# foolwood/SiamMask

Hardware: NVIDIA H100
Metric: search-region frames/sec (127/255 SiamMask-sharp) (higher is better)
Workload: dtype f16x3 (hi+lo split fp16 operands on wgmma, f32 accumulate; f32 CUDA-core xcorr/refine)

## Files before the change

siammask_b200/build.py:

```python
from __future__ import annotations

import os
import shutil
import subprocess
import sys

HERE = os.path.dirname(os.path.abspath(__file__))
CSRC = os.path.join(HERE, "csrc")
LIB = os.path.join(HERE, "libsiammask_b200.so")
SOURCES = ["conv_gemm_sm90.cu", "conv3x3_patch_sm90.cu", "stem_sm90.cu", "simt_kernels.cu", "xcorr_bulk.cu", "engine.cu"]
HEADERS = ["common.cuh", "ptx.cuh", os.path.join("..", "..", "include", "siammask_b200.h")]
NVCC_FLAGS = ["-gencode", "arch=compute_90a,code=sm_90a", "-lineinfo", "-O3", "-std=c++17",
              "-Xcompiler", "-fPIC", "-shared"]


def _nvcc() -> str:
    for cand in (os.environ.get("NVCC"), shutil.which("nvcc"), "/usr/local/cuda/bin/nvcc"):
        if cand and os.path.exists(cand):
            return cand
    raise RuntimeError("nvcc not found; cannot build libsiammask_b200.so")


HASH = LIB + ".srchash"


def source_hash() -> str:
    import hashlib
    h = hashlib.sha256(" ".join(NVCC_FLAGS).encode())
    for d in SOURCES + HEADERS:
        path = os.path.join(CSRC, d)
        h.update(d.encode())
        if os.path.exists(path):
            with open(path, "rb") as f:
                h.update(f.read())
    return h.hexdigest()


def is_stale() -> bool:
    if not os.path.exists(LIB):
        return True
    try:
        with open(HASH) as f:
            return f.read().strip() != source_hash()
    except OSError:
        return True


def build(force: bool = False, verbose: bool = False) -> str:
    if not force and not is_stale():
        return LIB
    tmp = f"{LIB}.tmp{os.getpid()}"
    cmd = [_nvcc(), *NVCC_FLAGS, "-o", tmp, *[os.path.join(CSRC, s) for s in SOURCES]]
    if verbose:
        print(" ".join(cmd), file=sys.stderr)
    digest = source_hash()
    res = subprocess.run(cmd, capture_output=True, text=True)
    if res.returncode != 0:
        if os.path.exists(tmp):
            os.remove(tmp)
        raise RuntimeError("nvcc failed:\n" + res.stdout + res.stderr)
    os.replace(tmp, LIB)
    with open(f"{HASH}.tmp{os.getpid()}", "w") as f:
        f.write(digest + "\n")
    os.replace(f"{HASH}.tmp{os.getpid()}", HASH)
    return LIB


if __name__ == "__main__":
    print(build(force="--force" in sys.argv, verbose=True))
```

siammask_b200/csrc/common.cuh:

```cuda
#pragma once
#include <cuda.h>
#include <cuda_fp16.h>
#include <cuda_runtime.h>
#include <cstdint>
#include <cstdio>
#include <stdexcept>
#include <string>
#include <vector>

struct sm_image_desc;

namespace smk {

struct Act {
  __half* hi = nullptr;
  __half* lo = nullptr;
  int B = 0, H = 0, W = 0, C = 0;
  int sexp = 0;
  __host__ __device__ size_t numel() const { return (size_t)B * H * W * C; }
  __host__ __device__ int M() const { return B * H * W; }
};

struct ConvGeom {
  int Cin, Cout, KH, KW, stride, pad, dil;
  __host__ __device__ int out_size(int in) const { return (in + 2 * pad - dil * (KH - 1) - 1) / stride + 1; }
};

enum OutMode : int { OUT_NHWC_SPLIT = 0, OUT_NHWC_F32 = 1, OUT_NCHW_F32 = 2 };

struct Epilogue {
  const float* alpha = nullptr;
  const float* beta = nullptr;
  const __half* res_hi = nullptr;
  const __half* res_lo = nullptr;
  float res_scale = 1.f;
  __half* out_hi = nullptr;
  __half* out_lo = nullptr;
  float* out_f32 = nullptr;
  int out_mode = OUT_NHWC_SPLIT;
  int relu = 0;
  int* ovf = nullptr;
};

__device__ __forceinline__ void flag_if_out_of_range(float absmax, int* ovf) {
  if (ovf != nullptr && !(absmax <= 65504.f)) atomicOr(ovf, 1);
}
constexpr int kStatusBadSlot = 2;

struct GemmSegment {
  CUtensorMap tmA[2];
  int mode;
  int num_kb, cblks, KW;
  int stride, pad, dil;
  int b_col0;
};

struct GemmParams {
  GemmSegment seg[2];
  int nseg;
  CUtensorMap tmB[2];
  CUtensorMap tmO[2];
  CUtensorMap tmR[2];
  int has_res;
  int M, Cout, Ho, Wo;
  int n_tiles, m_tiles;
  int reverse_m;
  Epilogue ep;
};

struct GemmInput {
  Act in;
  ConvGeom g;
  int w_col0;
};

struct TrackerHp {
  double context_amount, penalty_k, window_influence, lr;
  int32_t exemplar_size, instance_size, total_stride, base_size, out_size, reserved;
};

struct CudaError : std::runtime_error {
  using std::runtime_error::runtime_error;
};

#define SMK_CUDA(expr)                                                                              \
  do {                                                                                              \
    cudaError_t _e = (expr);                                                                        \
    if (_e != cudaSuccess)                                                                          \
      throw smk::CudaError(std::string(#expr) + " failed: " + cudaGetErrorString(_e) + " at " +    \
                           __FILE__ + ":" + std::to_string(__LINE__));                              \
  } while (0)

#define SMK_CHECK(cond, msg)                                                                        \
  do {                                                                                              \
    if (!(cond)) throw std::runtime_error(std::string("check failed: ") + #cond + " — " + (msg));   \
  } while (0)

template <typename K>
inline void ensure_dynamic_smem(K kernel, int bytes, unsigned long long& done_mask) {
  int dev = 0;
  SMK_CUDA(cudaGetDevice(&dev));
  const unsigned long long bit = 1ull << (dev & 63);
  if (done_mask & bit) return;
  SMK_CUDA(cudaFuncSetAttribute(kernel, cudaFuncAttributeMaxDynamicSharedMemorySize, bytes));
  done_mask |= bit;
}


bool gemm_conv_supported(const ConvGeom& g);
void launch_gemm_conv(const Act& in, const ConvGeom& g, const __half* w_hi, const __half* w_lo, int cout_pad,
                      const Epilogue& ep, int nsplit, int num_sms, cudaStream_t st);
void launch_gemm_multi(const GemmInput* convs, int nconv, const Act* residual, const __half* w_hi,
                       const __half* w_lo, int cout_pad, int w_ld, const Epilogue& ep, int nsplit, int num_sms,
                       cudaStream_t st, bool reverse_m = false);

CUtensorMap make_map_tiled_nd(const __half* base, int rank, const uint64_t* dims, const uint64_t* strides_bytes,
                              const uint32_t* box, int swizzle_bytes);

bool patch_conv_supported(const Act& in, const ConvGeom& g);
void launch_conv3x3_patch(const Act& in, const ConvGeom& g, const __half* w_hi, const __half* w_lo, int w_ld,
                          const Epilogue& ep, int nsplit, int num_sms, cudaStream_t st);

void launch_stem_tc(const float* x_nchw, int B, int S, const __half* w_hi, const __half* w_lo, const float* alpha,
                    const float* beta, Act out, int num_sms, cudaStream_t st, int* ovf = nullptr);

void launch_ref_conv(const Act& in, const ConvGeom& g, const float* w_krsc_cout, const Epilogue& ep,
                     cudaStream_t st);
void launch_stem(const float* x_nchw, int B, int S, const float* w, const float* alpha, const float* beta, Act out,
                 cudaStream_t st);
void launch_maxpool3s2(const Act& in, Act out, cudaStream_t st);
void launch_xcorr_nhwc(const Act& x, int c_off, const __half* k_hi, const __half* k_lo, int kh, int kw, Act out,
                       float mul, int* ovf, cudaStream_t st, const int32_t* slots = nullptr, int num_slots = 0);
void launch_scatter_slots(const __half* src_hi, const __half* src_lo, __half* dst_hi, __half* dst_lo,
                          const int32_t* slots, int B, int num_slots, int n, int* status, cudaStream_t st);
void launch_paste_labels(const float* masks, int side, const double* maps, const uint8_t* anno, const int32_t* obj_off,
                         const int32_t* objects, int G, int H, int W, double seg_thr, uint8_t* labels, cudaStream_t st,
                         const sm_image_desc* desc = nullptr);
void launch_paste_labels_iou(const float* masks, int side, const double* maps, const uint8_t* anno,
                             const int32_t* obj_off, const int32_t* objects, const int32_t* target_ids, int G, int H,
                             int W, double seg_thr, uint8_t* labels, const double* thrs, int T, int32_t* counts,
                             cudaStream_t st, const sm_image_desc* desc = nullptr);
void launch_label_boxes(const uint8_t* anno, int G, int H, int W, const int32_t* queries, int Q, int32_t* boxes,
                        cudaStream_t st, const sm_image_desc* desc = nullptr);
void launch_vot_overlap(const float* poly_a, const float* poly_b, int B, int W, int H, float* overlap, cudaStream_t st,
                        const int32_t* wh = nullptr);
void launch_vot_trajectory_overlap(const double* rec, int T, int S, const float* gt, int gt_frames, const int32_t* seq,
                                   const int32_t* wh, const int32_t* lengths, float* acc, float* eao, cudaStream_t st);
size_t vot_eao_workspace_size(int T, int S);
void launch_vot_eao_accumulate(const float* eao, const float* acc, const double* rec, int T, int S,
                               const int32_t* lengths, const int32_t* combo, int R, int cap, int tail_from,
                               const double* tail_in, double* tail_out, double* num, double* den, double* stats,
                               void* workspace, cudaStream_t st);
void launch_absmax(const Act& a, float* slot, cudaStream_t st);
void launch_xcorr_nchw_f32(const float* x, const float* k, float* out, int planes, int H, int W, int kh, int kw,
                           cudaStream_t st);
int launch_xcorr_bulk_f32(const float* x, const float* k, float* out, int planes, int H, int W, int kh, int kw,
                          cudaStream_t st);
void launch_crop_center(const Act& in, int crop, Act out, cudaStream_t st);
void launch_refine_crop(const Act& in, const int32_t* pos, int pos_max, int scale, int padv, int size, Act out,
                        cudaStream_t st);
void launch_gather_corr(const Act& corr, const int32_t* pos, float* out, float mul, cudaStream_t st);
void launch_gather_mask_col(const float* mask, const int32_t* pos, int B, int C, int R, float* out, cudaStream_t st);
void launch_deconv(const float* p3, const float* w, const float* bias, float* out, int B, int Cin, int N,
                   int cout, cudaStream_t st);
void launch_split_to_f32(const Act& in, float* out, cudaStream_t st, float mul = 1.f);
void launch_import_nchw(const float* x_nchw, Act out, cudaStream_t st);
void launch_warp_affine(const float* src, int sh, int sw, const double* maps, float* dst, int dh, int dw, float border,
                        int B, cudaStream_t st, const sm_image_desc* dst_desc = nullptr);
void launch_tracker_prepare(int B, const double* state, const int32_t* avg, const TrackerHp& hp, int32_t* boxes,
                            double* tsz, double* aux, cudaStream_t st);
void launch_tracker_update(int B, double* state, const float* rec, const double* aux, const int32_t* imsize,
                           const TrackerHp& hp, int A, int R, double* maps, double* out, cudaStream_t st,
                           const double* hp_table = nullptr);
void launch_crop_resize(const uint8_t* frames, size_t frame_stride, int H, int W, const int32_t* box, int B, int model,
                        float* out, cudaStream_t st, const int32_t* frame_idx = nullptr,
                        const sm_image_desc* desc = nullptr);
void launch_select(const float* cls, const float* loc, const float* anchors, const float* window, const double* tsz,
                   int B, int A, int R, double penalty_k, double window_influence, int32_t* best_idx, int32_t* pos,
                   float* rec, cudaStream_t st, const double* hp = nullptr);
void launch_mask_iou(const float* masks, int side, const double* maps, const uint8_t* anno, const int32_t* video, int B,
                     int H, int W, const double* thrs, int T, int32_t* counts, cudaStream_t st,
                     const sm_image_desc* desc = nullptr);
void launch_small_conv3x3_maps(const float* a, const float* b, int B, int Hi, int Wi, int Ho, int Wo, int Cin, int Cout,
                               const int* ymap, const int* xmap, const float* w, const float* bias, int relu,
                               float* out, cudaStream_t st);
std::vector<int> nearest_index_table(int out_size, int in_size);
int gemm_cout_pad(int cout);

}
```

siammask_b200/csrc/conv_gemm_sm90.cu:

```cuda
#include "common.cuh"
#include "ptx.cuh"

#include <cstdlib>
#include <cstring>
#include <mutex>
#include <unordered_map>

namespace smk {

namespace {

constexpr int BLOCK_M = 128;
constexpr int WG_ROWS = 64;
constexpr int CIN_GRAIN = 64;
constexpr int MMA_K = 16;
constexpr int SMEM_LIMIT = 227 * 1024;
constexpr int NUM_CONSUMER_WARPS = 8;
constexpr int NUM_THREADS = 128 + 32 * NUM_CONSUMER_WARPS;
constexpr int PRODUCER_REGS = 40;
constexpr int CONSUMER_REGS = 232;

template <int BLOCK_N, int NSPLIT>
struct Cfg {
  static constexpr int STAGING_BYTES = WG_ROWS * BLOCK_N * 4;
  static constexpr int RING_BYTES = SMEM_LIMIT - 2048 - 2 * STAGING_BYTES;
  static constexpr int stage_bytes(int bk) { return NSPLIT * (BLOCK_M + BLOCK_N) * bk * 2; }
  static constexpr int BLOCK_K = RING_BYTES / stage_bytes(64) >= 3 ? 64 : 32;
  static constexpr int SW = BLOCK_K * 2;
  static constexpr int A_TILE_BYTES = BLOCK_M * BLOCK_K * 2;
  static constexpr int B_TILE_BYTES = BLOCK_N * BLOCK_K * 2;
  static constexpr int STAGE_BYTES = NSPLIT * (A_TILE_BYTES + B_TILE_BYTES);
  static constexpr int RAW_STAGES = RING_BYTES / STAGE_BYTES;
  static constexpr int STAGES = RAW_STAGES > 6 ? 6 : RAW_STAGES;
  static constexpr int SMEM_BYTES = STAGES * STAGE_BYTES + 2 * STAGING_BYTES + 1024  + 256 ;
  static constexpr int ACC = BLOCK_N / 2;
  static constexpr int H_BOX = BLOCK_N < 64 ? BLOCK_N : 64;
  static constexpr int F_BOX = BLOCK_N < 32 ? BLOCK_N : 32;
  static constexpr int H_PLANE = WG_ROWS * BLOCK_N * 2;
  static_assert(STAGES >= 3, "pipeline needs at least three stages");
  static_assert(BLOCK_N % 16 == 0 && BLOCK_N >= 16 && BLOCK_N <= 128, "N tile (register accumulators)");
  static_assert(STAGE_BYTES % 1024 == 0 && B_TILE_BYTES % 1024 == 0, "stage parts stay 1024-aligned (swizzle atoms)");
  static_assert(SMEM_BYTES <= SMEM_LIMIT, "shared memory budget");
};

__device__ __forceinline__ int m_block(const GemmParams& p, int tile) {
  const int mb = tile / p.n_tiles;
  return p.reverse_m ? p.m_tiles - 1 - mb : mb;
}

template <int SPAN>
__device__ __forceinline__ uint32_t swizzle(uint32_t o) {
  return o ^ (((o >> 7) & (SPAN / 16 - 1)) << 4);
}

__device__ __forceinline__ void named_barrier_sync(int id, int threads) {
  asm volatile("bar.sync %0, %1;" ::"r"(id), "r"(threads) : "memory");
}

template <int BLOCK_N, int NSPLIT>
__global__ void __launch_bounds__(NUM_THREADS, 1) conv_gemm_kernel(const __grid_constant__ GemmParams p) {
  using C = Cfg<BLOCK_N, NSPLIT>;
  constexpr int STAGES = C::STAGES;
  constexpr int BLOCK_K = C::BLOCK_K;
  constexpr int A_TILE_BYTES = C::A_TILE_BYTES;

  extern __shared__ uint8_t smem_raw[];
  uint8_t* smem = smem_raw + ((1024u - (smem_u32(smem_raw) & 1023u)) & 1023u);
  uint8_t* staging = smem + STAGES * C::STAGE_BYTES;
  uint64_t* full_bar = reinterpret_cast<uint64_t*>(staging + 2 * C::STAGING_BYTES);
  uint64_t* empty_bar = full_bar + STAGES;
  uint64_t* free_bar = empty_bar + STAGES;
  uint64_t* res_bar = free_bar + 2;

  const int warp = __shfl_sync(0xffffffffu, (int)(threadIdx.x >> 5), 0);
  const int lane = threadIdx.x & 31;
  const int num_tiles = p.m_tiles * p.n_tiles;

  if (threadIdx.x == 0) {
    for (int i = 0; i < NSPLIT; ++i) {
      for (int sgi = 0; sgi < p.nseg; ++sgi) tma_prefetch_desc(&p.seg[sgi].tmA[i]);
      tma_prefetch_desc(&p.tmB[i]);
    }
    for (int s = 0; s < STAGES; ++s) {
      mbar_init(&full_bar[s], 1);
      mbar_init(&empty_bar[s], NUM_CONSUMER_WARPS);
    }
    for (int w = 0; w < 2; ++w) {
      mbar_init(&free_bar[w], 1);
      mbar_init(&res_bar[w], 1);
    }
    fence_barrier_init();
  }
  __syncthreads();

  if (warp < 4) {
    setmaxnreg_dec<PRODUCER_REGS>();
    if (warp != 0) return;
    const bool leader = elect_one();
    int stage = 0;
    uint32_t phase = 0;
    uint32_t iter = 0;
    for (int tile = blockIdx.x; tile < num_tiles; tile += gridDim.x, ++iter) {
      const int m0 = m_block(p, tile) * BLOCK_M;
      const int n0 = (tile % p.n_tiles) * BLOCK_N;
      const int q = m0 % p.Wo;
      const int t = m0 / p.Wo;
      const int pq = t % p.Ho;
      const int nb = t / p.Ho;
      for (int sgi = 0; sgi < p.nseg; ++sgi) {
        const GemmSegment& sg = p.seg[sgi];
        const int wb = q * sg.stride - sg.pad;
        const int hb = pq * sg.stride - sg.pad;
#pragma unroll 1
        for (int kb = 0; kb < sg.num_kb; ++kb) {
          mbar_wait(&empty_bar[stage], phase ^ 1);
          if (leader) mbar_arrive_expect_tx(&full_bar[stage], C::STAGE_BYTES);
          uint8_t* st = smem + stage * C::STAGE_BYTES;
          const int tap = kb / sg.cblks;
          const int c0 = (kb - tap * sg.cblks) * BLOCK_K;
#pragma unroll
          for (int s = 0; s < NSPLIT; ++s) {
            uint8_t* a_dst = st + s * A_TILE_BYTES;
            if (leader) {
              if (sg.mode == 0) {
                tma_load_2d(a_dst, &sg.tmA[s], &full_bar[stage], c0, m0);
              } else {
                const int r = tap / sg.KW;
                const int sx = tap - r * sg.KW;
                tma_load_im2col_4d(a_dst, &sg.tmA[s], &full_bar[stage], c0, wb, hb, nb,
                                   static_cast<uint16_t>(sx * sg.dil), static_cast<uint16_t>(r * sg.dil));
              }
              tma_load_2d(st + NSPLIT * A_TILE_BYTES + s * C::B_TILE_BYTES, &p.tmB[s], &full_bar[stage],
                          sg.b_col0 + kb * BLOCK_K, n0);
            }
          }
          __syncwarp();
          if (++stage == STAGES) { stage = 0; phase ^= 1; }
        }
      }
      if (p.has_res) {
#pragma unroll 1
        for (int w = 0; w < 2; ++w) {
          mbar_wait(&free_bar[w], iter & 1);
          const int r0 = m0 + w * WG_ROWS;
          if (leader) {
            mbar_arrive_expect_tx(&res_bar[w], r0 < p.M ? NSPLIT * C::H_PLANE : 0);
            if (r0 < p.M) {
              uint8_t* dst = staging + w * C::STAGING_BYTES;
#pragma unroll
              for (int s = 0; s < NSPLIT; ++s)
#pragma unroll
                for (int b = 0; b < BLOCK_N / C::H_BOX; ++b)
                  tma_load_2d(dst + s * C::H_PLANE + b * (WG_ROWS * C::H_BOX * 2), &p.tmR[s], &res_bar[w],
                              n0 + b * C::H_BOX, r0);
            }
          }
          __syncwarp();
        }
      }
    }
    return;
  }

  setmaxnreg_inc<CONSUMER_REGS>();
  const int wg = (warp >> 2) - 1;
  const int wl = warp & 3;
  const bool store_thread = wl == 0 && lane == 0;
  const Epilogue& ep = p.ep;
  const int HoWo = p.Ho * p.Wo;
  uint8_t* my_staging = staging + wg * C::STAGING_BYTES;
  float acc[C::ACC];
  float acc2[C::ACC];
  int stage = 0;
  uint32_t phase = 0;
  uint32_t iter = 0;
  for (int tile = blockIdx.x; tile < num_tiles; tile += gridDim.x, ++iter) {
#pragma unroll
    for (int i = 0; i < C::ACC; ++i) { acc[i] = 0.f; acc2[i] = 0.f; }
    int prev = -1;
    for (int sgi = 0; sgi < p.nseg; ++sgi) {
      const int nkb = p.seg[sgi].num_kb;
#pragma unroll 1
      for (int kb = 0; kb < nkb; ++kb) {
        mbar_wait(&full_bar[stage], phase);
        const uint32_t a_hi = smem_u32(smem + stage * C::STAGE_BYTES) + wg * (WG_ROWS * BLOCK_K * 2);
        const uint32_t b_hi = smem_u32(smem + stage * C::STAGE_BYTES) + NSPLIT * A_TILE_BYTES;
        const uint64_t da_hi0 = wgmma_desc_kmajor<C::SW>(a_hi);
        const uint64_t db_hi0 = wgmma_desc_kmajor<C::SW>(b_hi);
        const uint64_t da_lo0 = wgmma_desc_kmajor<C::SW>(a_hi + A_TILE_BYTES);
        const uint64_t db_lo0 = wgmma_desc_kmajor<C::SW>(b_hi + C::B_TILE_BYTES);
        wgmma_fence();
#pragma unroll
        for (int k = 0; k < BLOCK_K / MMA_K; ++k) {
          const uint64_t kadd = static_cast<uint64_t>(k * MMA_K * 2 / 16);
          wgmma_f16<BLOCK_N>(acc, da_hi0 + kadd, db_hi0 + kadd);
          if constexpr (NSPLIT == 2) {
            wgmma_f16<BLOCK_N>(acc2, da_hi0 + kadd, db_lo0 + kadd);
            wgmma_f16<BLOCK_N>(acc2, da_lo0 + kadd, db_hi0 + kadd);
          }
        }
        wgmma_commit();
        wgmma_wait<1>();
        if (prev >= 0) {
          __syncwarp();
          if (lane == 0) mbar_arrive(&empty_bar[prev]);
        } else if (store_thread) {
          tma_store_wait_read<0>();
          mbar_arrive(&free_bar[wg]);
        }
        prev = stage;
        if (++stage == STAGES) { stage = 0; phase ^= 1; }
      }
    }
    wgmma_wait<0>();
    fence_regs(acc);
    if constexpr (NSPLIT == 2) fence_regs(acc2);
    __syncwarp();
    if (lane == 0) mbar_arrive(&empty_bar[prev]);

    const int m0 = m_block(p, tile) * BLOCK_M + wg * WG_ROWS;
    const int n0 = (tile % p.n_tiles) * BLOCK_N;
    const int rl = wl * 16 + (lane >> 2);
    const int cl = 2 * (lane & 3);
    if (ep.out_mode == OUT_NCHW_F32) {
#pragma unroll
      for (int h = 0; h < 2; ++h) {
        const int m = m0 + rl + 8 * h;
        if (m >= p.M) continue;
        const int b = m / HoWo;
        const int hw = m - b * HoWo;
#pragma unroll
        for (int j = 0; j < BLOCK_N / 8; ++j) {
          const int n = n0 + cl + 8 * j;
          float v0 = acc[4 * j + 2 * h], v1 = acc[4 * j + 2 * h + 1];
          if constexpr (NSPLIT == 2) {
            v0 += acc2[4 * j + 2 * h];
            v1 += acc2[4 * j + 2 * h + 1];
          }
          const float2 al = __ldg(reinterpret_cast<const float2*>(ep.alpha + n));
          const float2 be = __ldg(reinterpret_cast<const float2*>(ep.beta + n));
          v0 = fmaf(v0, al.x, be.x);
          v1 = fmaf(v1, al.y, be.y);
          if (ep.relu) {
            v0 = fmaxf(v0, 0.f);
            v1 = fmaxf(v1, 0.f);
          }
          if (n < p.Cout) {
            float* dst = ep.out_f32 + (static_cast<size_t>(b) * p.Cout + n) * HoWo + hw;
            __stcs(dst, v0);
            if (n + 1 < p.Cout) __stcs(dst + HoWo, v1);
          }
        }
      }
      continue;
    }

    mbar_wait(p.has_res ? &res_bar[wg] : &free_bar[wg], iter & 1);
    const bool split = ep.out_mode == OUT_NHWC_SPLIT;
    const bool two_planes = ep.out_lo != nullptr;
    float amax = 0.f;
#pragma unroll
    for (int h = 0; h < 2; ++h) {
      const int r = rl + 8 * h;
      const bool row_in = m0 + r < p.M;
#pragma unroll
      for (int j = 0; j < BLOCK_N / 8; ++j) {
        const int c = cl + 8 * j;
        const int n = n0 + c;
        float v0 = acc[4 * j + 2 * h], v1 = acc[4 * j + 2 * h + 1];
        if constexpr (NSPLIT == 2) {
          v0 += acc2[4 * j + 2 * h];
          v1 += acc2[4 * j + 2 * h + 1];
        }
        const float2 al = __ldg(reinterpret_cast<const float2*>(ep.alpha + n));
        const float2 be = __ldg(reinterpret_cast<const float2*>(ep.beta + n));
        v0 = fmaf(v0, al.x, be.x);
        v1 = fmaf(v1, al.y, be.y);
        const uint32_t oh = (c / C::H_BOX) * (WG_ROWS * C::H_BOX * 2) +
                            swizzle<C::H_BOX * 2>(r * (C::H_BOX * 2) + (c % C::H_BOX) * 2);
        if (p.has_res) {
          float2 f = __half22float2(*reinterpret_cast<const __half2*>(my_staging + oh));
          if constexpr (NSPLIT == 2) {
            const float2 l = __half22float2(*reinterpret_cast<const __half2*>(my_staging + C::H_PLANE + oh));
            f.x += l.x;
            f.y += l.y;
          }
          v0 += f.x * ep.res_scale;
          v1 += f.y * ep.res_scale;
        }
        if (ep.relu) {
          v0 = fmaxf(v0, 0.f);
          v1 = fmaxf(v1, 0.f);
        }
        if (split) {
          if (row_in) amax = fmaxf(amax, fmaxf(fabsf(v0), fabsf(v1)));
          const __half2 hv = __floats2half2_rn(v0, v1);
          const float2 hf = __half22float2(hv);
          *reinterpret_cast<__half2*>(my_staging + oh) = hv;
          if (two_planes)
            *reinterpret_cast<__half2*>(my_staging + C::H_PLANE + oh) = __floats2half2_rn(v0 - hf.x, v1 - hf.y);
        } else {
          const uint32_t of = (c / C::F_BOX) * (WG_ROWS * C::F_BOX * 4) +
                              swizzle<C::F_BOX * 4>(r * (C::F_BOX * 4) + (c % C::F_BOX) * 4);
          *reinterpret_cast<float2*>(my_staging + of) = make_float2(v0, v1);
        }
      }
    }
    fence_proxy_async();
    named_barrier_sync(1 + wg, 128);
    if (store_thread && m0 < p.M) {
      if (split) {
        for (int s = 0; s < (two_planes ? 2 : 1); ++s)
#pragma unroll
          for (int b = 0; b < BLOCK_N / C::H_BOX; ++b)
            tma_store_2d(&p.tmO[s], my_staging + s * C::H_PLANE + b * (WG_ROWS * C::H_BOX * 2), n0 + b * C::H_BOX, m0);
      } else {
#pragma unroll
        for (int b = 0; b < BLOCK_N / C::F_BOX; ++b)
          tma_store_2d(&p.tmO[0], my_staging + b * (WG_ROWS * C::F_BOX * 4), n0 + b * C::F_BOX, m0);
      }
      tma_store_commit();
    }
    if (split) flag_if_out_of_range(amax, ep.ovf);
  }
  if (store_thread) tma_store_wait_all();
}

using EncodeTiledFn = CUresult (*)(CUtensorMap*, CUtensorMapDataType, cuuint32_t, void*, const cuuint64_t*,
                                   const cuuint64_t*, const cuuint32_t*, const cuuint32_t*, CUtensorMapInterleave,
                                   CUtensorMapSwizzle, CUtensorMapL2promotion, CUtensorMapFloatOOBfill);
using EncodeIm2colFn = CUresult (*)(CUtensorMap*, CUtensorMapDataType, cuuint32_t, void*, const cuuint64_t*,
                                    const cuuint64_t*, const int*, const int*, cuuint32_t, cuuint32_t,
                                    const cuuint32_t*, CUtensorMapInterleave, CUtensorMapSwizzle,
                                    CUtensorMapL2promotion, CUtensorMapFloatOOBfill);

struct DriverApi {
  EncodeTiledFn tiled = nullptr;
  EncodeIm2colFn im2col = nullptr;
  int driver_version = 0;
};

const DriverApi& driver_api() {
  static DriverApi api;
  static std::once_flag once;
  std::call_once(once, [] {
    void* fn = nullptr;
    cudaDriverEntryPointQueryResult q;
    SMK_CUDA(cudaGetDriverEntryPoint("cuTensorMapEncodeTiled", &fn, cudaEnableDefault, &q));
    SMK_CHECK(fn != nullptr && q == cudaDriverEntryPointSuccess, "cuTensorMapEncodeTiled not available");
    api.tiled = reinterpret_cast<EncodeTiledFn>(fn);
    fn = nullptr;
    SMK_CUDA(cudaGetDriverEntryPoint("cuTensorMapEncodeIm2col", &fn, cudaEnableDefault, &q));
    SMK_CHECK(fn != nullptr && q == cudaDriverEntryPointSuccess, "cuTensorMapEncodeIm2col not available");
    api.im2col = reinterpret_cast<EncodeIm2colFn>(fn);
    SMK_CUDA(cudaDriverGetVersion(&api.driver_version));
  });
  return api;
}

struct MapKey {
  uint64_t v[16];
  bool operator==(const MapKey& o) const { return std::memcmp(v, o.v, sizeof v) == 0; }
};
struct MapKeyHash {
  size_t operator()(const MapKey& k) const {
    uint64_t h = 0x9E3779B97F4A7C15ull;
    for (uint64_t x : k.v) { h ^= x + 0x9E3779B97F4A7C15ull + (h << 6) + (h >> 2); }
    return (size_t)h;
  }
};
template <typename F>
CUtensorMap cached_map(const MapKey& key, F&& encode) {
  static std::mutex mu;
  static std::unordered_map<MapKey, CUtensorMap, MapKeyHash> cache;
  int dev = 0;
  cudaGetDevice(&dev);
  MapKey k = key;
  k.v[15] = (uint64_t)dev;
  std::lock_guard<std::mutex> lock(mu);
  auto it = cache.find(k);
  if (it != cache.end()) return it->second;
  if (cache.size() > 65536) cache.clear();
  CUtensorMap m = encode();
  cache.emplace(k, m);
  return m;
}

CUtensorMap make_map_2d_raw(const __half* base, uint64_t inner, uint64_t outer, uint32_t box_inner, uint32_t box_outer) {
  CUtensorMap m;
  cuuint64_t dims[2] = {inner, outer};
  cuuint64_t strides[1] = {inner * sizeof(__half)};
  cuuint32_t box[2] = {box_inner, box_outer};
  cuuint32_t estr[2] = {1, 1};
  const CUtensorMapSwizzle sw = box_inner == 64 ? CU_TENSOR_MAP_SWIZZLE_128B : CU_TENSOR_MAP_SWIZZLE_64B;
  CUresult r = driver_api().tiled(&m, CU_TENSOR_MAP_DATA_TYPE_FLOAT16, 2, const_cast<__half*>(base), dims, strides,
                                  box, estr, CU_TENSOR_MAP_INTERLEAVE_NONE, sw,
                                  CU_TENSOR_MAP_L2_PROMOTION_L2_256B, CU_TENSOR_MAP_FLOAT_OOB_FILL_NONE);
  SMK_CHECK(r == CUDA_SUCCESS, "cuTensorMapEncodeTiled failed, code " + std::to_string((int)r));
  return m;
}

CUtensorMap make_map_2d(const __half* base, uint64_t inner, uint64_t outer, uint32_t box_inner, uint32_t box_outer) {
  MapKey k{};
  k.v[0] = 1; k.v[1] = (uint64_t)base; k.v[2] = inner; k.v[3] = outer; k.v[4] = box_inner; k.v[5] = box_outer;
  return cached_map(k, [&] { return make_map_2d_raw(base, inner, outer, box_inner, box_outer); });
}

CUtensorMap make_map_im2col_raw(const __half* base, const Act& in, const ConvGeom& g, int bk) {
  CUtensorMap m;
  cuuint64_t dims[4] = {(cuuint64_t)in.C, (cuuint64_t)in.W, (cuuint64_t)in.H, (cuuint64_t)in.B};
  cuuint64_t strides[3] = {(cuuint64_t)in.C * 2, (cuuint64_t)in.W * in.C * 2, (cuuint64_t)in.H * in.W * in.C * 2};
  int lower[2] = {-g.pad, -g.pad};
  int upper[2] = {g.pad - (g.KW - 1) * g.dil, g.pad - (g.KH - 1) * g.dil};
  cuuint32_t estr[4] = {1, (cuuint32_t)g.stride, (cuuint32_t)g.stride, 1};
  const DriverApi& api = driver_api();
  CUresult r = api.im2col(&m, CU_TENSOR_MAP_DATA_TYPE_FLOAT16, 4, const_cast<__half*>(base), dims, strides, lower,
                          upper, bk, BLOCK_M, estr, CU_TENSOR_MAP_INTERLEAVE_NONE,
                          bk == 64 ? CU_TENSOR_MAP_SWIZZLE_128B : CU_TENSOR_MAP_SWIZZLE_64B,
                          CU_TENSOR_MAP_L2_PROMOTION_L2_256B, CU_TENSOR_MAP_FLOAT_OOB_FILL_NONE);
  SMK_CHECK(r == CUDA_SUCCESS, "cuTensorMapEncodeIm2col failed, code " + std::to_string((int)r));
  if (api.driver_version <= 13010 && in.numel() * sizeof(__half) < 131072)
    reinterpret_cast<uint64_t*>(&m)[1] &= ~(1ull << 21);
  return m;
}

CUtensorMap make_map_im2col(const __half* base, const Act& in, const ConvGeom& g, int bk) {
  MapKey k{};
  k.v[0] = 3; k.v[1] = (uint64_t)base;
  k.v[2] = ((uint64_t)in.B << 32) | (uint32_t)in.H; k.v[3] = ((uint64_t)in.W << 32) | (uint32_t)in.C;
  k.v[4] = ((uint64_t)g.KH << 32) | (uint32_t)g.KW; k.v[5] = ((uint64_t)g.stride << 32) | (uint32_t)g.pad;
  k.v[6] = ((uint64_t)g.dil << 32) | (uint32_t)bk;
  return cached_map(k, [&] { return make_map_im2col_raw(base, in, g, bk); });
}

}

static CUtensorMap make_map_2d_any_raw(const __half* base, uint64_t inner, uint64_t outer, uint32_t box_inner, uint32_t box_outer,
                            int swizzle_bytes) {
  CUtensorMap m;
  cuuint64_t dims[2] = {inner, outer};
  cuuint64_t strides[1] = {inner * sizeof(__half)};
  cuuint32_t box[2] = {box_inner, box_outer};
  cuuint32_t estr[2] = {1, 1};
  const CUtensorMapSwizzle sw = swizzle_bytes == 128 ? CU_TENSOR_MAP_SWIZZLE_128B
                                : swizzle_bytes == 64 ? CU_TENSOR_MAP_SWIZZLE_64B : CU_TENSOR_MAP_SWIZZLE_32B;
  CUresult r = driver_api().tiled(&m, CU_TENSOR_MAP_DATA_TYPE_FLOAT16, 2, const_cast<__half*>(base), dims, strides,
                                  box, estr, CU_TENSOR_MAP_INTERLEAVE_NONE, sw, CU_TENSOR_MAP_L2_PROMOTION_L2_128B,
                                  CU_TENSOR_MAP_FLOAT_OOB_FILL_NONE);
  SMK_CHECK(r == CUDA_SUCCESS, "cuTensorMapEncodeTiled failed, code " + std::to_string((int)r));
  return m;
}

CUtensorMap make_map_2d_any(const __half* base, uint64_t inner, uint64_t outer, uint32_t box_inner, uint32_t box_outer,
                            int swizzle_bytes) {
  MapKey k{};
  k.v[0] = 5; k.v[1] = (uint64_t)base; k.v[2] = inner; k.v[3] = outer; k.v[4] = box_inner; k.v[5] = box_outer;
  k.v[6] = (uint64_t)swizzle_bytes;
  return cached_map(k, [&] { return make_map_2d_any_raw(base, inner, outer, box_inner, box_outer, swizzle_bytes); });
}

static CUtensorMap make_map_tiled_nd_raw(const __half* base, int rank, const uint64_t* dims,
                                         const uint64_t* strides_bytes, const uint32_t* box, int swizzle_bytes) {
  SMK_CHECK(rank >= 2 && rank <= 5, "tensor map rank");
  CUtensorMap m;
  cuuint64_t d[5], sb[4];
  cuuint32_t bx[5], es[5];
  for (int i = 0; i < rank; ++i) { d[i] = dims[i]; bx[i] = box[i]; es[i] = 1; }
  for (int i = 0; i + 1 < rank; ++i) sb[i] = strides_bytes[i];
  const CUtensorMapSwizzle sw = swizzle_bytes == 128 ? CU_TENSOR_MAP_SWIZZLE_128B
                                : swizzle_bytes == 64 ? CU_TENSOR_MAP_SWIZZLE_64B
                                : swizzle_bytes == 32 ? CU_TENSOR_MAP_SWIZZLE_32B : CU_TENSOR_MAP_SWIZZLE_NONE;
  CUresult r = driver_api().tiled(&m, CU_TENSOR_MAP_DATA_TYPE_FLOAT16, (cuuint32_t)rank, const_cast<__half*>(base), d, sb,
                                  bx, es, CU_TENSOR_MAP_INTERLEAVE_NONE, sw, CU_TENSOR_MAP_L2_PROMOTION_L2_256B,
                                  CU_TENSOR_MAP_FLOAT_OOB_FILL_NONE);
  SMK_CHECK(r == CUDA_SUCCESS, "cuTensorMapEncodeTiled (nd) failed, code " + std::to_string((int)r));
  return m;
}

CUtensorMap make_map_tiled_nd(const __half* base, int rank, const uint64_t* dims, const uint64_t* strides_bytes,
                              const uint32_t* box, int swizzle_bytes) {
  SMK_CHECK(rank >= 2 && rank <= 5, "tensor map rank");
  MapKey k{};
  k.v[0] = 4 | ((uint64_t)rank << 8) | ((uint64_t)swizzle_bytes << 16);
  k.v[1] = (uint64_t)base;
  for (int i = 0; i < rank; ++i) k.v[2 + i] = dims[i] | ((uint64_t)box[i] << 40);
  for (int i = 0; i + 1 < rank; ++i) k.v[7 + i] = strides_bytes[i];
  return cached_map(k, [&] { return make_map_tiled_nd_raw(base, rank, dims, strides_bytes, box, swizzle_bytes); });
}

bool gemm_conv_supported(const ConvGeom& g) { return g.Cin % CIN_GRAIN == 0 && g.Cout >= 1; }

int gemm_cout_pad(int cout) {
  if (cout <= 16) return 16;
  if (cout <= 32) return 32;
  if (cout <= 64) return 64;
  if (cout <= 128) return 128;
  return (cout + 255) / 256 * 256;
}

static CUtensorMap make_map_2d_f32(const float* base, uint64_t inner, uint64_t outer, uint32_t box_inner,
                                   uint32_t box_outer, int swizzle_bytes) {
  MapKey k{};
  k.v[0] = 6; k.v[1] = (uint64_t)base; k.v[2] = inner; k.v[3] = outer; k.v[4] = box_inner; k.v[5] = box_outer;
  k.v[6] = (uint64_t)swizzle_bytes;
  return cached_map(k, [&] {
    CUtensorMap m;
    cuuint64_t dims[2] = {inner, outer};
    cuuint64_t strides[1] = {inner * sizeof(float)};
    cuuint32_t box[2] = {box_inner, box_outer};
    cuuint32_t estr[2] = {1, 1};
    const CUtensorMapSwizzle sw = swizzle_bytes == 128 ? CU_TENSOR_MAP_SWIZZLE_128B
                                  : swizzle_bytes == 64 ? CU_TENSOR_MAP_SWIZZLE_64B : CU_TENSOR_MAP_SWIZZLE_32B;
    CUresult r = driver_api().tiled(&m, CU_TENSOR_MAP_DATA_TYPE_FLOAT32, 2, const_cast<float*>(base), dims, strides,
                                    box, estr, CU_TENSOR_MAP_INTERLEAVE_NONE, sw, CU_TENSOR_MAP_L2_PROMOTION_L2_128B,
                                    CU_TENSOR_MAP_FLOAT_OOB_FILL_NONE);
    SMK_CHECK(r == CUDA_SUCCESS, "cuTensorMapEncodeTiled (f32) failed, code " + std::to_string((int)r));
    return m;
  });
}

template <int BLOCK_N, int NSPLIT>
static void launch_cfg(GemmParams& p, const GemmInput* convs, const __half* w_hi, const __half* w_lo, int cout_pad,
                       int w_ld, int num_sms, cudaStream_t st) {
  using C = Cfg<BLOCK_N, NSPLIT>;
  constexpr int bk = C::BLOCK_K;
  for (int i = 0; i < p.nseg; ++i) {
    const ConvGeom& g = convs[i].g;
    const Act& in = convs[i].in;
    GemmSegment& sg = p.seg[i];
    sg.cblks = g.Cin / bk;
    sg.num_kb = g.KH * g.KW * sg.cblks;
    for (int s = 0; s < NSPLIT; ++s) {
      const __half* a = s == 0 ? in.hi : in.lo;
      sg.tmA[s] = sg.mode == 0 ? make_map_2d(a, g.Cin, (uint64_t)in.M(), bk, BLOCK_M) : make_map_im2col(a, in, g, bk);
    }
    if (NSPLIT == 1) sg.tmA[1] = sg.tmA[0];
  }
  if (p.nseg == 1) p.seg[1] = p.seg[0];
  for (int s = 0; s < NSPLIT; ++s) p.tmB[s] = make_map_2d(s == 0 ? w_hi : w_lo, (uint64_t)w_ld, cout_pad, bk, BLOCK_N);
  if (NSPLIT == 1) p.tmB[1] = p.tmB[0];

  auto kern = conv_gemm_kernel<BLOCK_N, NSPLIT>;
  static unsigned long long attr_done = 0;
  ensure_dynamic_smem(kern, C::SMEM_BYTES, attr_done);
  const int tiles = p.m_tiles * p.n_tiles;
  const int grid = tiles < num_sms ? tiles : num_sms;
  kern<<<grid, NUM_THREADS, C::SMEM_BYTES, st>>>(p);
  SMK_CUDA(cudaGetLastError());
}

void launch_gemm_conv(const Act& in, const ConvGeom& g, const __half* w_hi, const __half* w_lo, int cout_pad,
                      const Epilogue& ep, int nsplit, int num_sms, cudaStream_t st) {
  GemmInput gi{in, g, 0};
  launch_gemm_multi(&gi, 1, nullptr, w_hi, w_lo, cout_pad, g.KH * g.KW * g.Cin, ep, nsplit, num_sms, st);
}

void launch_gemm_multi(const GemmInput* convs, int nconv, const Act* residual, const __half* w_hi,
                       const __half* w_lo, int cout_pad, int w_ld, const Epilogue& ep, int nsplit, int num_sms,
                       cudaStream_t st, bool reverse_m) {
  SMK_CHECK(nconv >= 1 && nconv <= 2, "1 or 2 convolution segments");
  const ConvGeom& g0 = convs[0].g;
  const Act& in0 = convs[0].in;
  const int Ho = g0.out_size(in0.H), Wo = g0.out_size(in0.W);
  GemmParams p;
  std::memset(&p, 0, sizeof p);
  p.M = in0.B * Ho * Wo;
  p.Cout = g0.Cout;
  p.Ho = Ho;
  p.Wo = Wo;
  const int block_n = cout_pad < 128 ? cout_pad : 128;
  SMK_CHECK(cout_pad % block_n == 0, "cout_pad must be a multiple of the N tile");
  if (ep.out_mode != OUT_NCHW_F32) SMK_CHECK(g0.Cout == cout_pad, "NHWC outputs need Cout to match the padded tile width");
  p.n_tiles = cout_pad / block_n;
  p.m_tiles = (p.M + BLOCK_M - 1) / BLOCK_M;
  p.reverse_m = reverse_m ? 1 : 0;
  p.nseg = nconv;
  for (int i = 0; i < nconv; ++i) {
    const ConvGeom& g = convs[i].g;
    const Act& in = convs[i].in;
    SMK_CHECK(gemm_conv_supported(g), "Cin must be a multiple of 64 for the tensor-core conv");
    SMK_CHECK(in.C == g.Cin && g.Cout == g0.Cout && in.B == in0.B, "segment channels/batch mismatch");
    SMK_CHECK(g.out_size(in.H) == Ho && g.out_size(in.W) == Wo, "segments must produce the same output size");
    SMK_CHECK(nsplit == 1 || (in.lo != nullptr && w_lo != nullptr), "exact mode needs lo planes");
    GemmSegment& sg = p.seg[i];
    sg.KW = g.KW;
    sg.stride = g.stride;
    sg.pad = g.pad;
    sg.dil = g.dil;
    sg.mode = (g.KH == 1 && g.KW == 1 && g.stride == 1 && g.pad == 0) ? 0 : 1;
    sg.b_col0 = convs[i].w_col0;
    SMK_CHECK(sg.b_col0 % 64 == 0 && sg.b_col0 + g.KH * g.KW * g.Cin <= w_ld, "weight column range");
  }
  const uint32_t hbox = block_n < 64 ? block_n : 64, fbox = block_n < 32 ? block_n : 32;
  auto aligned = [](const void* q) { return (reinterpret_cast<uintptr_t>(q) & 15) == 0; };
  if (ep.out_mode == OUT_NHWC_SPLIT) {
    SMK_CHECK(aligned(ep.out_hi) && (ep.out_lo == nullptr || aligned(ep.out_lo)), "NHWC output planes 16-byte aligned");
    for (int s = 0; s < (ep.out_lo != nullptr ? 2 : 1); ++s)
      p.tmO[s] = make_map_2d_any(s == 0 ? ep.out_hi : ep.out_lo, (uint64_t)p.Cout, (uint64_t)p.M, hbox, 64, hbox * 2);
  } else if (ep.out_mode == OUT_NHWC_F32) {
    SMK_CHECK(aligned(ep.out_f32), "NHWC fp32 output 16-byte aligned");
    p.tmO[0] = make_map_2d_f32(ep.out_f32, (uint64_t)p.Cout, (uint64_t)p.M, fbox, 64, fbox * 4);
  }
  if (residual != nullptr) {
    SMK_CHECK(ep.out_mode == OUT_NHWC_SPLIT, "a residual needs an NHWC split-plane output");
    SMK_CHECK(residual->C == g0.Cout && residual->M() == p.M, "residual shape");
    SMK_CHECK(nsplit == 1 || residual->lo != nullptr, "exact mode residual needs both planes");
    SMK_CHECK(aligned(residual->hi) && (nsplit == 1 || aligned(residual->lo)), "residual planes 16-byte aligned");
    p.has_res = 1;
    for (int s = 0; s < nsplit; ++s)
      p.tmR[s] = make_map_2d_any(s == 0 ? residual->hi : residual->lo, (uint64_t)p.Cout, (uint64_t)p.M, hbox, 64,
                                 hbox * 2);
  }
  p.ep = ep;

#define SMK_DISPATCH(BN)                                                                         \
  case BN:                                                                                       \
    if (nsplit == 2) launch_cfg<BN, 2>(p, convs, w_hi, w_lo, cout_pad, w_ld, num_sms, st);       \
    else launch_cfg<BN, 1>(p, convs, w_hi, w_lo, cout_pad, w_ld, num_sms, st);                   \
    break;
  switch (block_n) {
    SMK_DISPATCH(16)
    SMK_DISPATCH(32)
    SMK_DISPATCH(64)
    SMK_DISPATCH(128)
    default: SMK_CHECK(false, "unsupported N tile");
  }
#undef SMK_DISPATCH
}

}
```

Baseline: 4630.

## Add weight-resident wgmma kernel for 1x1 NCHW fp32 head convolutions

Adds a specialized warp-specialized wgmma kernel for 1x1 stride-1 convolutions that write NCHW fp32 output. Each CTA keeps the whole K extent of a 128-wide weight tile resident in shared memory and streams only activation tiles through a deep TMA ring. Two consumer warpgroups alternate over 64-row M tiles, and the generic GEMM launcher routes matching single-conv calls here. This is meant to avoid reloading weights per tile and to use smaller M tiles that spread the head layers over more SMs. The cost is extra barrier complexity, and the kernel only applies to Cin values whose weights fit in 128 KB.

```diff
diff --git a/siammask_b200/build.py b/siammask_b200/build.py
--- a/siammask_b200/build.py
+++ b/siammask_b200/build.py
@@ -8,7 +8,7 @@
 HERE = os.path.dirname(os.path.abspath(__file__))
 CSRC = os.path.join(HERE, "csrc")
 LIB = os.path.join(HERE, "libsiammask_b200.so")
-SOURCES = ["conv_gemm_sm90.cu", "conv3x3_patch_sm90.cu", "stem_sm90.cu", "simt_kernels.cu", "xcorr_bulk.cu", "engine.cu"]
+SOURCES = ["conv_gemm_sm90.cu", "head_nchw_sm90.cu", "conv3x3_patch_sm90.cu", "stem_sm90.cu", "simt_kernels.cu", "xcorr_bulk.cu", "engine.cu"]
 HEADERS = ["common.cuh", "ptx.cuh", os.path.join("..", "..", "include", "siammask_b200.h")]
 NVCC_FLAGS = ["-gencode", "arch=compute_90a,code=sm_90a", "-lineinfo", "-O3", "-std=c++17",
               "-Xcompiler", "-fPIC", "-shared"]
diff --git a/siammask_b200/csrc/common.cuh b/siammask_b200/csrc/common.cuh
--- a/siammask_b200/csrc/common.cuh
+++ b/siammask_b200/csrc/common.cuh
@@ -114,6 +114,10 @@
                        const __half* w_lo, int cout_pad, int w_ld, const Epilogue& ep, int nsplit, int num_sms,
                        cudaStream_t st, bool reverse_m = false);
 
+bool head_nchw_supported(const ConvGeom& g, int cout_pad, int out_mode, int nsplit);
+void launch_head_nchw(GemmParams p, const GemmInput& conv, const __half* w_hi, const __half* w_lo, int cout_pad,
+                      int w_ld, int nsplit, int num_sms, cudaStream_t st);
+
 CUtensorMap make_map_tiled_nd(const __half* base, int rank, const uint64_t* dims, const uint64_t* strides_bytes,
                               const uint32_t* box, int swizzle_bytes);
 
diff --git a/siammask_b200/csrc/conv_gemm_sm90.cu b/siammask_b200/csrc/conv_gemm_sm90.cu
--- a/siammask_b200/csrc/conv_gemm_sm90.cu
+++ b/siammask_b200/csrc/conv_gemm_sm90.cu
@@ -612,6 +612,10 @@
                                  hbox * 2);
   }
   p.ep = ep;
+  if (nconv == 1 && residual == nullptr && head_nchw_supported(g0, cout_pad, ep.out_mode, nsplit)) {
+    launch_head_nchw(p, convs[0], w_hi, w_lo, cout_pad, w_ld, nsplit, num_sms, st);
+    return;
+  }
 
 #define SMK_DISPATCH(BN)                                                                         \
   case BN:                                                                                       \
diff --git a/siammask_b200/csrc/head_nchw_sm90.cu b/siammask_b200/csrc/head_nchw_sm90.cu
--- /dev/null
+++ b/siammask_b200/csrc/head_nchw_sm90.cu
@@ -0,0 +1,249 @@
+#include "common.cuh"
+#include "ptx.cuh"
+
+namespace smk {
+
+namespace {
+
+constexpr int ROWS = 64;
+constexpr int BLOCK_N = 128;
+constexpr int BLOCK_K = 64;
+constexpr int MMA_K = 16;
+constexpr int SMEM_LIMIT = 227 * 1024;
+constexpr int NUM_THREADS = 384;
+constexpr int PRODUCER_REGS = 40;
+constexpr int CONSUMER_REGS = 232;
+constexpr int W_BYTES = 128 * 1024;
+constexpr int BAR_WEIGHTS = 1;
+constexpr int BAR_TURN = 2;
+
+template <int NSPLIT>
+struct HeadCfg {
+  static constexpr int B_BOX = BLOCK_N * BLOCK_K * 2;
+  static constexpr int A_BOX = ROWS * BLOCK_K * 2;
+  static constexpr int KB_MAX = W_BYTES / (NSPLIT * B_BOX);
+  static constexpr int STAGE_BYTES = NSPLIT * A_BOX;
+  static constexpr int RAW_STAGES = (SMEM_LIMIT - W_BYTES - 1024 - 256) / STAGE_BYTES;
+  static constexpr int STAGES = RAW_STAGES > 8 ? 8 : RAW_STAGES;
+  static constexpr int SMEM_BYTES = W_BYTES + STAGES * STAGE_BYTES + 1024  + 256 ;
+  static constexpr int ACC = BLOCK_N / 2;
+  static_assert(STAGES >= 4, "ring depth");
+  static_assert(SMEM_BYTES <= SMEM_LIMIT, "shared memory budget");
+};
+
+__device__ __forceinline__ void bar_sync(int id, int threads) {
+  asm volatile("bar.sync %0, %1;" ::"r"(id), "r"(threads) : "memory");
+}
+__device__ __forceinline__ void bar_arrive(int id, int threads) {
+  asm volatile("bar.arrive %0, %1;" ::"r"(id), "r"(threads) : "memory");
+}
+
+__device__ __forceinline__ void item_range(int items, int& first, int& end) {
+  const int cta = blockIdx.x, per = items / (int)gridDim.x, extra = items % (int)gridDim.x;
+  first = cta * per + min(cta, extra);
+  end = first + per + (cta < extra ? 1 : 0);
+}
+
+template <int NSPLIT>
+__global__ void __launch_bounds__(NUM_THREADS, 1) head_nchw_kernel(const __grid_constant__ GemmParams p) {
+  using C = HeadCfg<NSPLIT>;
+  constexpr int STAGES = C::STAGES;
+
+  extern __shared__ uint8_t smem_raw[];
+  uint8_t* smem = smem_raw + ((1024u - (smem_u32(smem_raw) & 1023u)) & 1023u);
+  uint8_t* wts = smem;
+  uint8_t* ring = smem + W_BYTES;
+  uint64_t* full_bar = reinterpret_cast<uint64_t*>(ring + STAGES * C::STAGE_BYTES);
+  uint64_t* empty_bar = full_bar + STAGES;
+  uint64_t* w_bar = empty_bar + STAGES;
+
+  const int warp = __shfl_sync(0xffffffffu, (int)(threadIdx.x >> 5), 0);
+  const int lane = threadIdx.x & 31;
+  const GemmSegment& sg = p.seg[0];
+  const int nkb = sg.num_kb;
+  const int m_tiles = p.m_tiles;
+  int first, end;
+  item_range(m_tiles * p.n_tiles, first, end);
+
+  if (threadIdx.x == 0) {
+    for (int i = 0; i < NSPLIT; ++i) {
+      tma_prefetch_desc(&sg.tmA[i]);
+      tma_prefetch_desc(&p.tmB[i]);
+    }
+    for (int s = 0; s < STAGES; ++s) {
+      mbar_init(&full_bar[s], 1);
+      mbar_init(&empty_bar[s], 4);
+    }
+    mbar_init(w_bar, 1);
+    fence_barrier_init();
+  }
+  __syncthreads();
+
+  if (warp < 4) {
+    setmaxnreg_dec<PRODUCER_REGS>();
+    if (warp != 0) return;
+    const bool leader = elect_one();
+    int stage = 0;
+    uint32_t phase = 0;
+    for (int i = first; i < end; ++i) {
+      const int nt = i / m_tiles;
+      const int mb = i - nt * m_tiles;
+      const int m0 = (p.reverse_m ? m_tiles - 1 - mb : mb) * ROWS;
+      if (i == first || mb == 0) {
+        if (i > first) bar_sync(BAR_WEIGHTS, 32 + 256);
+        if (leader) {
+          mbar_arrive_expect_tx(w_bar, NSPLIT * nkb * C::B_BOX);
+#pragma unroll 1
+          for (int kb = 0; kb < nkb; ++kb)
+#pragma unroll
+            for (int s = 0; s < NSPLIT; ++s)
+              tma_load_2d(wts + (s * C::KB_MAX + kb) * C::B_BOX, &p.tmB[s], w_bar, sg.b_col0 + kb * BLOCK_K,
+                          nt * BLOCK_N);
+        }
+        __syncwarp();
+      }
+#pragma unroll 1
+      for (int kb = 0; kb < nkb; ++kb) {
+        mbar_wait(&empty_bar[stage], phase ^ 1);
+        if (leader) {
+          mbar_arrive_expect_tx(&full_bar[stage], C::STAGE_BYTES);
+#pragma unroll
+          for (int s = 0; s < NSPLIT; ++s)
+            tma_load_2d(ring + stage * C::STAGE_BYTES + s * C::A_BOX, &sg.tmA[s], &full_bar[stage], kb * BLOCK_K, m0);
+        }
+        __syncwarp();
+        if (++stage == STAGES) { stage = 0; phase ^= 1; }
+      }
+    }
+    return;
+  }
+
+  setmaxnreg_inc<CONSUMER_REGS>();
+  const int wg = (warp >> 2) - 1;
+  const int wl = warp & 3;
+  const Epilogue& ep = p.ep;
+  const int HoWo = p.Ho * p.Wo;
+  const int rl = wl * 16 + (lane >> 2);
+  const int cl = 2 * (lane & 3);
+  float acc[C::ACC];
+  float acc2[C::ACC];
+  for (int i = first + wg;; i += 2) {
+    for (int b = i - 1; b <= i && b < end; ++b)
+      if (b > first && b % m_tiles == 0) bar_sync(BAR_WEIGHTS, 32 + 256);
+    if (i >= end) break;
+    const int nt = i / m_tiles;
+    const int mb = i - nt * m_tiles;
+    if (i > first) bar_sync(BAR_TURN + wg, 256);
+    mbar_wait(w_bar, (nt - first / m_tiles) & 1);
+#pragma unroll
+    for (int r = 0; r < C::ACC; ++r) { acc[r] = 0.f; acc2[r] = 0.f; }
+    int prev = -1;
+#pragma unroll 1
+    for (int kb = 0; kb < nkb; ++kb) {
+      const int g = (i - first) * nkb + kb;
+      const int stage = g % STAGES;
+      mbar_wait(&full_bar[stage], (g / STAGES) & 1);
+      const uint32_t a_hi = smem_u32(ring + stage * C::STAGE_BYTES);
+      const uint32_t b_hi = smem_u32(wts + kb * C::B_BOX);
+      const uint64_t da_hi0 = wgmma_desc_kmajor<128>(a_hi);
+      const uint64_t db_hi0 = wgmma_desc_kmajor<128>(b_hi);
+      const uint64_t da_lo0 = wgmma_desc_kmajor<128>(a_hi + C::A_BOX);
+      const uint64_t db_lo0 = wgmma_desc_kmajor<128>(b_hi + C::KB_MAX * C::B_BOX);
+      wgmma_fence();
+#pragma unroll
+      for (int k = 0; k < BLOCK_K / MMA_K; ++k) {
+        const uint64_t kadd = static_cast<uint64_t>(k * MMA_K * 2 / 16);
+        wgmma_f16<BLOCK_N>(acc, da_hi0 + kadd, db_hi0 + kadd);
+        if constexpr (NSPLIT == 2) {
+          wgmma_f16<BLOCK_N>(acc2, da_hi0 + kadd, db_lo0 + kadd);
+          wgmma_f16<BLOCK_N>(acc2, da_lo0 + kadd, db_hi0 + kadd);
+        }
+      }
+      wgmma_commit();
+      wgmma_wait<1>();
+      if (prev >= 0) {
+        __syncwarp();
+        if (lane == 0) mbar_arrive(&empty_bar[prev]);
+      }
+      prev = stage;
+    }
+    if (i + 1 < end) bar_arrive(BAR_TURN + (wg ^ 1), 256);
+    wgmma_wait<0>();
+    fence_regs(acc);
+    if constexpr (NSPLIT == 2) fence_regs(acc2);
+    __syncwarp();
+    if (lane == 0) mbar_arrive(&empty_bar[prev]);
+
+    const int m0 = (p.reverse_m ? m_tiles - 1 - mb : mb) * ROWS;
+    const int n0 = nt * BLOCK_N;
+    float* row[2];
+#pragma unroll
+    for (int h = 0; h < 2; ++h) {
+      const int m = m0 + rl + 8 * h;
+      const int b = m / HoWo;
+      row[h] = m < p.M ? ep.out_f32 + static_cast<size_t>(b) * p.Cout * HoWo + (m - b * HoWo) : nullptr;
+    }
+#pragma unroll
+    for (int c = 0; c < BLOCK_N / 8; ++c) {
+      const int n = n0 + cl + 8 * c;
+      const float2 al = __ldg(reinterpret_cast<const float2*>(ep.alpha + n));
+      const float2 be = __ldg(reinterpret_cast<const float2*>(ep.beta + n));
+#pragma unroll
+      for (int h = 0; h < 2; ++h) {
+        float v0 = acc[4 * c + 2 * h], v1 = acc[4 * c + 2 * h + 1];
+        if constexpr (NSPLIT == 2) {
+          v0 += acc2[4 * c + 2 * h];
+          v1 += acc2[4 * c + 2 * h + 1];
+        }
+        v0 = fmaf(v0, al.x, be.x);
+        v1 = fmaf(v1, al.y, be.y);
+        if (ep.relu) {
+          v0 = fmaxf(v0, 0.f);
+          v1 = fmaxf(v1, 0.f);
+        }
+        if (row[h] != nullptr && n < p.Cout) {
+          float* dst = row[h] + static_cast<size_t>(n) * HoWo;
+          __stcs(dst, v0);
+          if (n + 1 < p.Cout) __stcs(dst + HoWo, v1);
+        }
+      }
+    }
+  }
+}
+
+}
+
+CUtensorMap make_map_2d_any(const __half* base, uint64_t inner, uint64_t outer, uint32_t box_inner, uint32_t box_outer,
+                            int swizzle_bytes);
+
+bool head_nchw_supported(const ConvGeom& g, int cout_pad, int out_mode, int nsplit) {
+  const int k_max = W_BYTES / (nsplit * BLOCK_N * 2);
+  return out_mode == OUT_NCHW_F32 && g.KH == 1 && g.KW == 1 && g.stride == 1 && g.pad == 0 && cout_pad >= BLOCK_N &&
+         cout_pad % BLOCK_N == 0 && g.Cin % BLOCK_K == 0 && g.Cin <= k_max;
+}
+
+void launch_head_nchw(GemmParams p, const GemmInput& conv, const __half* w_hi, const __half* w_lo, int cout_pad,
+                      int w_ld, int nsplit, int num_sms, cudaStream_t st) {
+  const Act& in = conv.in;
+  SMK_CHECK(head_nchw_supported(conv.g, cout_pad, p.ep.out_mode, nsplit), "geometry not supported by the head kernel");
+  GemmSegment& sg = p.seg[0];
+  sg.num_kb = conv.g.Cin / BLOCK_K;
+  for (int s = 0; s < nsplit; ++s) {
+    sg.tmA[s] = make_map_2d_any(s == 0 ? in.hi : in.lo, (uint64_t)conv.g.Cin, (uint64_t)in.M(), BLOCK_K, ROWS, 128);
+    p.tmB[s] = make_map_2d_any(s == 0 ? w_hi : w_lo, (uint64_t)w_ld, (uint64_t)cout_pad, BLOCK_K, BLOCK_N, 128);
+  }
+  p.n_tiles = cout_pad / BLOCK_N;
+  p.m_tiles = (p.M + ROWS - 1) / ROWS;
+  const int items = p.m_tiles * p.n_tiles;
+  const int grid = items < num_sms ? items : num_sms;
+  auto go = [&](auto kern, int smem_bytes, unsigned long long& attr_done) {
+    ensure_dynamic_smem(kern, smem_bytes, attr_done);
+    kern<<<grid, NUM_THREADS, smem_bytes, st>>>(p);
+    SMK_CUDA(cudaGetLastError());
+  };
+  static unsigned long long attr_exact = 0, attr_fast = 0;
+  if (nsplit == 2) go(head_nchw_kernel<2>, HeadCfg<2>::SMEM_BYTES, attr_exact);
+  else go(head_nchw_kernel<1>, HeadCfg<1>::SMEM_BYTES, attr_fast);
+}
+
+}
```

After: 4692, median of 6. 1.01x the previous value.
